# seryrzu/centroFlye

Measured on AMD Instinct MI355X. Metric: long-read bases/sec through rare-k-mer recruit+distance, higher is better.
Workload: dtype u8 bases -> u64 k-mers / u32 indices (integer only)

## Files before the change

### centroflye_amd/csrc/hip/cf_api.hip

```cpp
#include "cf_common.h"

#include <atomic>
#include <cstdlib>
#include <mutex>
#include <thread>

#ifndef CF_COPY_MODE_DEFAULT
#define CF_COPY_MODE_DEFAULT 1
#endif
struct alignas(16) cf_u32x4_api { uint32_t x, y, z, w; };

int cf_fail(cf_ctx* ctx, int code, const std::string& msg) {
    if (ctx) ctx->err = msg;
    return code;
}


static std::mutex g_pool_lock;
static std::vector<cf_ctx*> g_contexts;

static void cf_pool_flush_locked(cf_ctx* ctx) {
    for (auto& kv : ctx->pool) { ctx->block_bytes.erase(kv.second); (void)hipFree(kv.second); }
    ctx->pool.clear();
    ctx->pooled = 0;
// ... 457 lines not shown
        ctx->dist_hot_entries = (int)value;
    } else if (n == "lut_shift") {
        if (value < -1 || value > 3) return cf_fail(ctx, -22, "lut_shift out of range (-1 = by the set's size, 0 .. 3)");
        ctx->lut_shift = (int)value;
    } else if (n == "dist_regions") {
        if (value != 0 && value != 1 && value != 2 && value != 4 && value != 8) return cf_fail(ctx, -22, "dist_regions must be 0 (auto), 1, 2, 4 or 8");
        ctx->dist_regions = (int)value;
    } else if (n == "dist_dbits") {
        if (value != 0 && (value < 5 || value > 8)) return cf_fail(ctx, -22, "dist_dbits must be 0 (auto) or 5 .. 8");
        ctx->dist_dbits = (int)value;
    } else if (n == "dist_fill_pct") {
        if (value < 10 || value > 90) return cf_fail(ctx, -22, "dist_fill_pct out of range (10 .. 90)");
        ctx->dist_fill_pct = (int)value;
    } else if (n == "dist_edge_chunk") {
        if (value < 0 || value > (1 << 20)) return cf_fail(ctx, -22, "dist_edge_chunk out of range (0 = default, 1 .. 2^20)");
        ctx->dist_edge_chunk = (int)value;
    } else if (n == "dist_int_thr") {
        ctx->dist_int_thr = value != 0;
    } else if (n == "dist_sketch_bits") {
        if (value != 0 && value != 4 && value != 8) return cf_fail(ctx, -22, "dist_sketch_bits must be 0 (by min_cov), 4 or 8");
        ctx->dist_sketch_bits = (int)value;
    } else if (n == "dist_sketch_tail") {
        ctx->dist_sketch_tail = value != 0;
    } else if (n == "dist_classes") {
        ctx->dist_classes = value != 0;
    } else if (n == "dist_class_bits") {
        if (value < 1 || value > 16) return cf_fail(ctx, -22, "dist_class_bits out of range (1 .. 16)");
        ctx->dist_class_bits = (int)value;
    } else if (n == "dist_groups") {
        ctx->dist_groups = value != 0;
    } else if (n == "dist_group_cap") {
        if (value < 1 || value > 32) return cf_fail(ctx, -22, "dist_group_cap out of range (1 .. 32)");
        ctx->dist_group_cap = (int)value;
    } else if (n == "dist_sketch") {
        ctx->dist_sketch = value != 0;
    } else if (n == "dist_est_pct") {
        if (value < 5 || value > 100) return cf_fail(ctx, -22, "dist_est_pct out of range (5 .. 100)");
        ctx->dist_est_pct = (int)value;
    } else if (n == "dist_stage") {
        if (value < 0 || value > 2048) return cf_fail(ctx, -22, "dist_stage out of range (0 .. 2048)");
        ctx->dist_stage = (int)value;
    } else if (n == "place_fused") {
        ctx->place_fused = value != 0;
    } else if (n == "dist_region_bytes") {
        ctx->dist_region_bytes = value != 0;
    } else if (n == "place_mode") {
        if (value < 1 || value > 3) return cf_fail(ctx, -22, "place_mode out of range (1 = hash map, 2 = per-read regions unless min_inters < 4, 3 = per-read regions always)");
        ctx->place_mode = (int)value;
    } else if (n == "place_block") {
        if (value != 0 && (value < 128 || value > 1024 || value % 128)) return cf_fail(ctx, -22, "place_block must be 0 or a multiple of 128 in 128 .. 1024");
        ctx->place_block = (int)value;
    } else if (n == "place_row_words") {
        if (value != 0 && value != 32 && value != 64) return cf_fail(ctx, -22, "place_row_words must be 0 (auto), 32 or 64");
        ctx->place_row_words = (int)value;
    } else if (n == "place_l3") {
        if (value < 0 || value > 2) return cf_fail(ctx, -22, "place_l3 must be 0 (auto), 1 (always) or 2 (never)");
        ctx->place_l3 = (int)value;
    } else if (n == "place_l3_shift") {
        if (value < 0 || value > 6) return cf_fail(ctx, -22, "place_l3_shift must be 0 (= 6) .. 6");
        ctx->place_l3_shift = (int)value;
    } else if (n == "place_long_rescans") {
        if (value < -1 || value > 1000000) return cf_fail(ctx, -22, "place_long_rescans out of range (-1, 0 .. 1000000)");
        ctx->place_long_rescans = (int)value;
    } else if (n == "place_cmap_bits") {
        if (value < 0 || value > 30) return cf_fail(ctx, -22, "place_cmap_bits out of range (0 = default, 1 .. 30)");
        ctx->place_cmap_bits = (int)value;
// ... 85 lines not shown
```

### centroflye_amd/csrc/hip/cf_common.h

```cpp
#pragma once
#include <hip/hip_runtime.h>

#include <algorithm>
#include <cstdint>
#include <cstdio>
#include <cstring>
#include <map>
#include <string>
#include <unordered_map>
#include <vector>

#include "cfhip.h"

extern __shared__ __attribute__((aligned(16))) unsigned char cf_lds[];

#define CF_WAVE 64

#ifndef cf_lds_at
typedef __attribute__((address_space(3))) unsigned char cf_lds_u8;
__device__ __forceinline__ unsigned char* cf_lds_at(uint32_t off) { return (unsigned char*)((cf_lds_u8*)(uintptr_t)(off + 16u) - 16); }
__device__ __forceinline__ bool cf_lds_base_ok() { return (uint32_t)(uintptr_t)(cf_lds_u8*)cf_lds == 0u; }
#endif

__device__ __forceinline__ uint64_t cf_mix64(uint64_t x) {
// ... 114 lines not shown
    std::vector<cf_monodec_read> monodec_reads;
    std::vector<int64_t> monodec_ptr;
    std::vector<cf_monodec_inst> monodec_inst;
    cf_monodec_shape monodec_last{};

    static constexpr int kCopyThreads = 16;
    void* pin_slot[kCopyThreads] = {nullptr};
    hipStream_t pin_stream[kCopyThreads] = {nullptr};
    size_t pin_bytes = 0;
    int copy_threads = 16;

    cf_stats stats{};
    cf_times times{};

    int dist_block = 0;
    int dist_wgs = 0;
    int dist_slots = 0;
    int dist_wide = 0;
    int dist_post_atomics = 0;
    int dist_hot_cap = 0;
    int lut_shift = -1;
    int dist_hot_entries = 32768;
    int dist_regions = 0;
    int dist_region_bytes = 0;
    int dist_dbits = 0;
    int dist_fill_pct = 70;
    int dist_edge_chunk = 0;
    int dist_int_thr = 1;
    int dist_sketch = 1;
    bool dist_sketch_tail = true;
    int dist_class_bits = 16;
    bool dist_classes = true;
    bool dist_groups = true;
    int dist_group_cap = 32;
    int dist_sketch_bits = 0;
    int dist_est_pct = 80;
    int dist_stage = 2048;
    int place_chunk = 2, place_grid = 0;
    int place_fused = 1;
    int place_mode = 2;
    int place_block = 0;
    int place_row_words = 0;
    int place_long_rescans = 2;
    int place_cmap_bits = 0;
    int place_slots_per_unit = 0;
    int place_l3 = 0;
    int place_l3_shift = 0;
    int map_window = 0;
    int edit_lds_diags = 0;
    int tandem_key_mode = 0;
    int64_t tandem_batch_windows = 0;
    int64_t cons_batch_bytes = 0;
    int64_t ualign_batch_bytes = 0;
    int64_t monodec_batch_bytes = 0;
    int count_mode = 1;
    int count_bits = 0;
    int count_slots = 4096;
    int count_tile = 16;
    int count_skip_exotic = 0;
    int64_t comm_round_bytes = (int64_t)256 << 20;
    int comm_self_p2p = 0;
};

int cf_fail(cf_ctx* ctx, int code, const std::string& msg);
int cf_copy_h2d(cf_ctx* ctx, void* dev, const void* host, size_t bytes);
int cf_copy_d2h(cf_ctx* ctx, void* host, const void* dev, size_t bytes);
// ... 84 lines not shown
```

### centroflye_amd/csrc/hip/cf_dist.hip

```cpp
#include "cf_common.h"

#include <cstdlib>

void cf_free_edges(cf_ctx* c);
int cf_refresh_unique_count(cf_ctx* ctx);

#define DIST_STAGE_CAP 1024
#define DIST_STACK 112
#define DIST_UNROLL 4
#define DIST_ITEM (64u * DIST_UNROLL)
#define DIST_BM_BITS 65536u
#define DIST_HOT_CAP 2048u
#define DIST_EDGE_CHUNK 8192ull
#define DIST_OVQ 160u
#define DIST_LDS_HEAD (DIST_BM_BITS / 8 + 128)
#define DIST_CNT_MASK 0x7FFFFFu
#define DIST_SEL_BIT (1ull << 23)

#ifndef cf_ballot
__device__ __forceinline__ unsigned long long cf_ballot(bool p) { return __builtin_amdgcn_ballot_w64(p); }
#endif

struct alignas(16) cf_dist_rec { uint32_t e0; uint32_t len; uint32_t ig; uint32_t nu; };

__global__ void __launch_bounds__(256)
cf_post_hist_kernel(const int32_t* __restrict__ entries, int64_t e0, int64_t e1, uint32_t part, uint32_t n_parts, uint32_t* __restrict__ cnt) {
    const int64_t stride = (int64_t)gridDim.x * blockDim.x;
    for (int64_t i = e0 + (int64_t)blockIdx.x * blockDim.x + threadIdx.x; i < e1; i += stride) {
        const uint32_t x = (uint32_t)entries[i];
        if (n_parts == 1u || x % n_parts == part) atomicAdd(&cnt[x], 1u);
    }
}

__global__ void __launch_bounds__(256)
cf_post_fill_kernel(const int64_t* __restrict__ cloud_ptr, const int32_t* __restrict__ entries, int64_t u0, int64_t u1, uint32_t part, uint32_t n_parts,
                    const int64_t* __restrict__ post_ptr, uint32_t* __restrict__ cursor, int32_t* __restrict__ post,
                    uint32_t* __restrict__ first_unit) {
    const int lane = threadIdx.x & 63;
    const int64_t wave = ((int64_t)blockIdx.x * blockDim.x + threadIdx.x) >> 6;
    const int64_t n_waves = ((int64_t)gridDim.x * blockDim.x) >> 6;
    for (int64_t u = u0 + wave; u < u1; u += n_waves) {
        const int64_t a = cloud_ptr[u], b = cloud_ptr[u + 1];
        for (int64_t e = a + lane; e < b; e += 64) {
            const int32_t x = entries[e];
            if (n_parts != 1u && (uint32_t)x % n_parts != part) continue;
// ... 336 lines not shown
struct alignas(8) cf_dist_item { uint32_t e, m; };
#ifndef CF_DIST_ITEMS_BLOCKED
#define CF_DIST_ITEMS_BLOCKED 0
#endif
struct alignas(16) cf_dist_head { uint32_t a, n_items; unsigned long long ibase; uint32_t n_entries, n_useful, n_members, first_member; };

struct cf_dist_args {
    const int64_t* post_ptr;
    const int32_t* post;
    const int64_t* cloud_ptr;
    const int32_t* entries;
    const int32_t* unit_rend;
    const int32_t* unit_rbeg;
    const cf_dist_rec* urange;
    const uint16_t* entry_i;
    const uint8_t* entry_i8;
    uint32_t reg_shift;
    const uint32_t* packed;
    int64_t n_kmers;
    int32_t part, n_parts;
    int32_t min_d, max_d;
    uint32_t min_cov;
    double thr;
    uint32_t thr_num, thr_den;
    int32_t slots;
    uint32_t fill_limit;
    uint32_t est_limit;
    int32_t sketch;
    uint32_t sk_counters, sk_shift, sk_mask;
    uint32_t sk_fbits, sk_fsh, sk_wshift, sk_fmask, sk_guard, sk_bytes;
    const cf_dist_head* heads;
    const cf_dist_item* items;
    uint32_t stage_cap;
    uint32_t hot_cap;
    uint32_t hot_entries;
    uint32_t* edges;
    unsigned long long edge_cap;
    const uint32_t* member_mask;
    const int32_t* order;
    int64_t n_order;
    unsigned long long edge_chunk;
    unsigned long long* holes;
    unsigned long long* counters;
    uint32_t* unique_bits;
};

typedef uint32_t cf_raw4 __attribute__((ext_vector_type(4)));
struct __attribute__((packed, aligned(4))) cf_run4 { uint32_t x, y, z, w; };
__device__ __forceinline__ void cf_load_packed4(const cf_dist_args& A, uint32_t s_e, uint32_t l4, uint32_t& x, uint32_t& y, uint32_t& z, uint32_t& w) {
#if !defined(CF_NO_BUFFER_LOAD)
    const __amdgpu_buffer_rsrc_t rs = __builtin_amdgcn_make_buffer_rsrc((void*)A.packed, 0, (int)0xFFFFFFFFu, 0x00020000);
    const cf_raw4 v = __builtin_amdgcn_raw_buffer_load_b128(rs, (int)(l4 * 4u), (int)(s_e << 2), 0);
    x = v.x; y = v.y; z = v.z; w = v.w;
#else
    const uint32_t* p = A.packed + s_e;
    const cf_run4 r = *(const cf_run4*)(p + l4);
    x = r.x; y = r.y; z = r.z; w = r.w;
#endif
}

struct alignas(16) cf_u64x2 { unsigned long long x, y; };
struct alignas(16) cf_u32x4 { uint32_t x, y, z, w; };

template <int DB>
struct cf_tab_wide_t {
    static constexpr uint32_t kCntBits = 31 - DB, kCntMask = (1u << kCntBits) - 1u, kDMask = (1u << DB) - 1u, kDShift = 32 - DB;
// ... 451 lines not shown
        if (!(m.w[0] | m.w[1] | m.w[2] | m.w[3])) return;
        const bucket k = this->read(bk);
#pragma unroll
        for (int i = 0; i < 4; ++i) {
            const uint32_t cnt = cnt_of(m.w[i]);
            if (cnt >= min_cov && k.k[i] != kEmpty) {
                const uint32_t b = k.k[i] & kBMask;
                const unsigned long long total = (k.k[3] == kEmpty && N::home(N::hash(b), n_buckets) == bk) ? (unsigned long long)sum_of(k, m, b) : total_of(b, n_buckets);
                f(4u * bk + (uint32_t)i, b, k.k[i] >> kBBits, cnt, total);
            }
        }
    }
    static constexpr uint32_t kScanGroup = 4;
    static __device__ __forceinline__ uint32_t slot_of_bit(uint32_t bit) { return bit; }
    __device__ __forceinline__ uint32_t hot_mask(uint32_t g, uint32_t min_cov) const {
        const masks m = read_masks(g);
        const uint32_t need = max(min_cov, 1u);
        return (uint32_t)(all_of(m.w[0]) >= need) | ((uint32_t)(all_of(m.w[1]) >= need) << 1) | ((uint32_t)(all_of(m.w[2]) >= need) << 2) | ((uint32_t)(all_of(m.w[3]) >= need) << 3);
    }
    template <class F>
    __device__ __forceinline__ void eval_slot(uint32_t s, uint32_t n_buckets, uint32_t min_cov, F&& f) const {
        const uint32_t bk = s >> 2, i = s & 3u;
        const bucket k = this->read(bk);
        const masks m = read_masks(bk);
        uint32_t mine = k.k[0], mine_m = m.w[0];
#pragma unroll
        for (int j = 1; j < 4; ++j) { if (i == (uint32_t)j) { mine = k.k[j]; mine_m = m.w[j]; } }
        const uint32_t cnt = cnt_of(mine_m);
        if (mine == kEmpty || cnt < min_cov) return;
        const uint32_t b = mine & kBMask;
        const unsigned long long total = (k.k[3] == kEmpty && N::home(N::hash(b), n_buckets) == bk) ? (unsigned long long)sum_of(k, m, b) : total_of(b, n_buckets);
        f(s, b, mine >> kBBits, cnt, total);
    }
    template <class F>
    __device__ __forceinline__ void for_marked(uint32_t bk, F&& f) const {
        const uint32_t w = (mk[bk >> 3] >> ((bk & 7u) * 4u)) & 15u;
        if (!w) return;
        const bucket k = this->read(bk);
        const masks m = read_masks(bk);
#pragma unroll
        for (int i = 0; i < 4; ++i)
            if ((w >> i) & 1u) f(4u * bk + (uint32_t)i, k.k[i] & kBMask, k.k[i] >> kBBits, cnt_of(m.w[i]));
    }
    __device__ __forceinline__ void mark(uint32_t s) const { atomicOr(&mk[s >> 5], 1u << (s & 31u)); }
    __device__ __forceinline__ void unmark(uint32_t s) const { atomicAnd(&mk[s >> 5], ~(1u << (s & 31u))); }
};

struct cf_tab_region {
    static constexpr int PB = 4;
    static constexpr uint32_t kBBits = 24, kBMask = (1u << kBBits) - 1u;
    static constexpr uint32_t kSlotBytes = 6, kPerBucket = PB, kAll = (1u << PB) - 1u;
    static constexpr bool kMaskTab = false;
    static constexpr uint32_t kEmpty = 0xFFFFFFFFu;
    struct bucket { uint32_t k[PB]; };
    struct counts { uint32_t w[PB / 2]; };
    struct raw { uint32_t b, i; };
    typedef unsigned long long qitem;
    uint32_t* keys;
    uint32_t* cnt32;
    uint32_t S, nb_r;
    __device__ __forceinline__ void init(unsigned char* lds, uint32_t slots) { keys = (uint32_t*)lds; cnt32 = keys + slots; S = 0; nb_r = slots / PB; }
    __device__ __forceinline__ void configure(const cf_dist_args& A, uint32_t n_buckets) { S = A.reg_shift; nb_r = n_buckets >> A.reg_shift; }
    __device__ __forceinline__ void clear(uint32_t slots, uint32_t t, uint32_t nt) const {
        const cf_u32x4 e{kEmpty, kEmpty, kEmpty, kEmpty}, z{0u, 0u, 0u, 0u};
        for (uint32_t s = t; s < (slots >> 2); s += nt) ((cf_u32x4*)keys)[s] = e;
        for (uint32_t s = t; s < (slots >> 3); s += nt) ((cf_u32x4*)cnt32)[s] = z;
// ... 504 lines not shown
#ifndef CF_DIST_PF_B
#define CF_DIST_PF_B 1
#endif

#ifndef CF_DIST_LB_THREADS
#define CF_DIST_LB_THREADS 1024
#define CF_DIST_LB_BLOCKS 1
#endif
template <class Tab, bool CLS>
__global__ void __launch_bounds__(CF_DIST_LB_THREADS, CF_DIST_LB_BLOCKS) cf_dist_kernel(cf_dist_args A) {
    const int t = threadIdx.x, lane = t & 63, nt = blockDim.x;
    uint32_t* bm = (uint32_t*)cf_lds_at(0u);
    uint32_t* sh = bm + DIST_BM_BITS / 32;
    unsigned char* lds_tab = cf_lds_at(DIST_LDS_HEAD);
    Tab T;
    T.init(lds_tab, (uint32_t)A.slots);
    T.configure(A, (uint32_t)A.slots / Tab::kPerBucket);
    uint32_t* sk = (uint32_t*)lds_tab;
    size_t tab_bytes = (size_t)A.slots * Tab::kSlotBytes;
    if constexpr (Tab::kMaskTab) tab_bytes += Tab::extra_bytes((uint32_t)A.slots);
    uint16_t* stage = (uint16_t*)(lds_tab + tab_bytes);
    uint32_t* stack = (uint32_t*)(stage + DIST_STAGE_CAP + 8);
    typename Tab::qitem* wq0 = (typename Tab::qitem*)(stack + 2 * DIST_STACK);
    const uint32_t wv = (uint32_t)__builtin_amdgcn_readfirstlane((int)(t >> 6)), nw = (uint32_t)nt >> 6;
    typename Tab::qitem* wq = wq0 + (size_t)wv * DIST_QSTRIDE;
    typename Tab::qitem* ovq = wq0 + (size_t)(nt >> 6) * DIST_QSTRIDE + (size_t)wv * DIST_OVQ;
    uint16_t* hotl = (uint16_t*)(wq0 + (size_t)(nt >> 6) * (DIST_QSTRIDE + DIST_OVQ));
    uint8_t* wqb = (uint8_t*)(hotl + DIST_HOT_CAP) + (size_t)wv * (DIST_QSTRIDE + DIST_OVQ);
    uint8_t* ovqb = wqb + DIST_QSTRIDE;
    const uint32_t slots = (uint32_t)A.slots, n_buckets = slots / Tab::kPerBucket;
    unsigned long long acc_E = 0, acc_spill = 0, acc_pass = 0, acc_edges = 0;
#if defined(CF_DIST_DIAG_COUNT)
    unsigned long long dg_swept = 0;
    unsigned long long dg[8] = {0, 0, 0, 0, 0, 0, 0, 0};
#define CF_DG(X) X
#define CF_DG_PTR (&dg[0])
#else
#define CF_DG(X)
#define CF_DG_PTR nullptr
#endif
#if defined(CF_DIST_STAMPS)
    unsigned long long stamp_acc[8] = {0, 0, 0, 0, 0, 0, 0, 0}, stamp_t = __builtin_amdgcn_s_memtime();
#endif

    const int64_t q_per = (A.n_order + 7) / 8;
    auto pop_issue = [&]() -> unsigned long long { return atomicAdd(&A.counters[16 + 16 * (blockIdx.x & 7)], 1ull); };
    auto pop_finish = [&](unsigned long long q) -> long long {
        const int x0 = (int)(blockIdx.x & 7);
        const int64_t lo0 = x0 * q_per, hi0 = min((int64_t)(x0 + 1) * q_per, A.n_order);
        if (lo0 + (int64_t)q < hi0) return lo0 + (int64_t)q;
        for (int s8 = 1; s8 < 8; ++s8) {
            const int x = (int)((blockIdx.x + s8) & 7);
            const int64_t lo = x * q_per, hi = min((int64_t)(x + 1) * q_per, A.n_order);
            if (lo >= hi) continue;
            const unsigned long long q2 = atomicAdd(&A.counters[16 + 16 * x], 1ull);
            if (lo + (int64_t)q2 < hi) return lo + (int64_t)q2;
        }
        return -1;
    };
    long long nx_idx = -1;
    cf_dist_head nx_head{0u, 0u, 0ull, 0u, 0u, 1u, 0u};
    unsigned long long nx_q = 0;
    if (!cf_lds_base_ok()) { if (t == 0) atomicOr(&A.counters[4], 2ull); return; }
    auto publish_next = [&]() {
        sh[16] = (uint32_t)(unsigned long long)nx_idx; sh[17] = (uint32_t)((unsigned long long)nx_idx >> 32);
        sh[18] = nx_head.a; sh[19] = nx_head.n_items; sh[20] = (uint32_t)nx_head.ibase; sh[21] = (uint32_t)(nx_head.ibase >> 32);
// ... 90 lines not shown
                            for (int u = 0; u < DIST_UNROLL; ++u)
                                if (seen_[u] >= m_guard && ((ok >> u) & 1u)) atomicSub(&sk[sft_[u] >> 5], 1u << (sft_[u] & 31u));
                        }
                        if (seen_max == m_fmask) sh[m_flag] = 1u;
                    }
                    return false;
                });
                CF_STAMP(6);
            }
            __syncthreads();
            CF_STAMP(7);
            if (!sh[m_flag]) break;
            if (m_fbits == 8u) { mark_all = true; break; }
            m_fbits = 8u; m_fsh = 3u; m_wshift = 2u; m_fmask = 255u; m_guard = 0x7FFFFFFFu; m_shift = A.sk_shift + 1u; m_flag = 31u;
            }
        }
        if (t == 0) { nx_idx = pop_finish(nx_q); if (nx_idx >= 0) nx_head = A.heads[nx_idx]; }
        if (mark_all) {
            const cf_u32x4 ones{0xFFFFFFFFu, 0xFFFFFFFFu, 0xFFFFFFFFu, 0xFFFFFFFFu};
            for (uint32_t s = (uint32_t)t; s < DIST_BM_BITS / 128; s += (uint32_t)nt) ((cf_u32x4*)bm)[s] = ones;
            if (t == 0) {
                uint32_t P0 = 1;
                while (P0 < 64u && (unsigned long long)n_ent_a > (unsigned long long)A.est_limit * P0) P0 <<= 1;
                for (uint32_t i = 0; i < P0; ++i) { stack[2 * i] = P0; stack[2 * i + 1] = i; }
                sh[2] = P0;
                pop_pass();
            }
        }
        bool spilled = false;
        if (CF_DIST_ABL < 7) T.clear(slots, (uint32_t)t, (uint32_t)nt);
        __syncthreads();
        while (true) {
            const uint32_t P = sh[3], pidx = sh[4], pmask = P - 1u;
            uint32_t my_e = 0, s_e = 0;
            CF_STAMP(2);
            {
                uint32_t qtail = 0, otail = 0;
                bool too_full = sh[0] > A.fill_limit;
#if CF_DIST_HOTBLK
                uint32_t hcur = 0, hend = 0;
#define CF_DIST_HOT(SLOT) {                                                                                   \
                    const unsigned long long hm_ = cf_ballot((SLOT) != 0xFFFFFFFFu);                           \
                    if (hm_ && use_hot) {       \
                        const uint32_t hn_ = (uint32_t)__popcll(hm_), room_ = hend - hcur;                    \
                        uint32_t hp_ = hcur + cf_rank_in(hm_);                                                \
                        if (hn_ > room_) {       \
                            uint32_t nb_ = 0;                                                                 \
                            if (lane == 0) nb_ = atomicAdd(&sh[11], 64u);                                     \
                            nb_ = (uint32_t)__builtin_amdgcn_readfirstlane((int)nb_);                         \
                            if (nb_ + (uint32_t)lane < DIST_HOT_CAP) hotl[nb_ + (uint32_t)lane] = (uint16_t)0xFFFFu; \
                            hp_ = hp_ < hend ? hp_ : nb_ + (hp_ - hend);                                      \
                            hcur = nb_ + (hn_ - room_); hend = nb_ + 64u;                                     \
                        } else hcur += hn_;                                                                   \
                        if ((SLOT) != 0xFFFFFFFFu && hp_ < DIST_HOT_CAP) hotl[hp_] = (uint16_t)(SLOT);        \
                    }                                                                                         \
                }
#elif defined(CF_DIST_DIAG_NOHOT)
#define CF_DIST_HOT(SLOT) { if ((SLOT) == 0xFFFFFFF0u) sh[11] = 1u; }
#else
#define CF_DIST_HOT(SLOT) {                                                                                   \
                    const unsigned long long hm_ = cf_ballot((SLOT) != 0xFFFFFFFFu);                           \
                    if (hm_ && use_hot) {                                                                     \
                        uint32_t hb_ = 0;                                                                     \
                        if (lane == 0) hb_ = atomicAdd(&sh[11], (uint32_t)__popcll(hm_));                     \
                        hb_ = (uint32_t)__builtin_amdgcn_readfirstlane((int)hb_) + cf_rank_in(hm_);          \
                        if ((SLOT) != 0xFFFFFFFFu && hb_ < DIST_HOT_CAP) hotl[hb_] = (uint16_t)(SLOT);        \
// ... 201 lines not shown
            const uint32_t n_groups = slots / Tab::kScanGroup;
            for (uint32_t g0 = 0; g0 < n_groups; g0 += (uint32_t)nt) {
                const uint32_t bk = g0 + (uint32_t)t;
                const uint32_t m = bk < n_groups ? T.hot_mask(bk, A.min_cov) : 0u;
                const uint32_t cnt = (uint32_t)__popc(m);
                if (cf_ballot(cnt != 0u)) {
                    uint32_t total = 0;
                    for (uint32_t k = 0; k < Tab::kScanGroup; ++k) { const unsigned long long bk_ = cf_ballot(cnt > k); if (!bk_) break; total += (uint32_t)__popcll(bk_); }
                    uint32_t base = 0;
                    if (lane == 0) base = atomicAdd(&sh[11], total);
                    base = (uint32_t)__builtin_amdgcn_readfirstlane((int)base);
                    uint32_t mm = m;
                    for (uint32_t k = 0; k < Tab::kScanGroup; ++k) {
                        const unsigned long long bk_ = cf_ballot(cnt > k);
                        if (!bk_) break;
                        if (cnt > k) {
                            const uint32_t bit = (uint32_t)__ffs((int)mm) - 1u;
                            mm &= mm - 1u;
                            const uint32_t pos = base + cf_rank_in(bk_);
                            if (pos < hot_cap) hot[pos] = (uint16_t)(Tab::kScanGroup * bk + Tab::slot_of_bit(bit));
                        }
                        base += (uint32_t)__popcll(bk_);
                    }
                }
            }
            __syncthreads();
            }
            const uint32_t n_hot = sh[11];
            auto dominant = [&](uint32_t cnt, unsigned long long total) -> bool {
                if (A.thr_den) return (unsigned long long)A.thr_den * cnt >= (unsigned long long)A.thr_num * total;
                return ((double)cnt / (double)total) >= A.thr;
            };
            uint32_t sel_prev = 0, sp_left = 0;
            for (uint32_t mj = 0; mj < n_mem; ++mj) {
                const uint32_t am = mj ? (uint32_t)A.order[(size_t)m_first + mj] : a;
                if constexpr (Tab::kMaskTab) T.set_member(A.member_mask[(size_t)m_first + mj], T.counting);
                const unsigned long long ch_base = ((unsigned long long)sh[29] << 32) | sh[28];
                const uint32_t ch_rows = sh[27];
                auto put_row = [&](unsigned long long o, uint32_t b, uint32_t dd, uint32_t cnt) {
                    if (o < A.edge_cap) *(cf_u32x4*)(A.edges + 4 * o) = cf_u32x4{dd, am, b, cnt};
                    const uint32_t bit = 1u << (b & 31);
                    if (!(A.unique_bits[b >> 5] & bit)) atomicOr(&A.unique_bits[b >> 5], bit);
                };
                auto set_unique = [&](uint32_t w, uint32_t b) { const uint32_t bit = 1u << (b & 31); if (!(w & bit)) atomicOr(&A.unique_bits[b >> 5], bit); };
                auto keep = [&](bool sel, uint32_t s, uint32_t b, uint32_t dd, uint32_t cnt) -> bool {
                    const unsigned long long m = cf_ballot(sel);
                    if (!m) return false;
                    uint32_t row0 = 0;
                    if (lane == 0) { const uint32_t n = (uint32_t)__popcll(m); atomicAdd(&sh[8], n); row0 = atomicAdd(&sh[26], n); }
                    const uint32_t row = (uint32_t)__builtin_amdgcn_readfirstlane((int)row0) + (uint32_t)__popcll(m & lt);
                    const bool late = sel && row >= ch_rows;
                    const unsigned long long o = ch_base + row;
                    if (sel && !late && o < A.edge_cap) *(cf_u32x4*)(A.edges + 4 * o) = cf_u32x4{dd, am, b, cnt};
                    const unsigned long long ml = cf_ballot(late);
                    if (ml) {
                        uint32_t p0 = 0;
                        if (lane == 0) p0 = atomicAdd(&sh[30], (uint32_t)__popcll(ml));
                        const uint32_t pos = (uint32_t)__builtin_amdgcn_readfirstlane((int)p0) + (uint32_t)__popcll(ml & lt);
                        if (late) { T.mark(s); if (pos < A.stage_cap) stage[pos] = (uint16_t)s; }
                    }
                    return sel && !late;
                };
                if (CF_DIST_ABL >= 1) { }
                else if (n_hot <= hot_cap) {
                    bool p_on = false;
                    uint32_t p_w = 0, p_b = 0;
                    for (uint32_t i0 = 0; i0 < n_hot; i0 += (uint32_t)nt) {
                        const uint32_t i = i0 + (uint32_t)t;
                        bool sel = false;
                        uint32_t s = 0, eb = 0, ed = 0, ec = 0;
                        if (i < n_hot && (s = hot[i]) != 0xFFFFu) {
                            T.eval_slot(s, n_buckets, A.min_cov, [&](uint32_t, uint32_t b, uint32_t dd, uint32_t cnt, unsigned long long total) { sel = b != am && dominant(cnt, total); eb = b; ed = dd; ec = cnt; });
                        }
                        const bool wrote = keep(sel, s, eb, ed, ec);
                        uint32_t w_new = 0;
                        if (wrote) w_new = A.unique_bits[eb >> 5];
                        if (p_on) set_unique(p_w, p_b);
                        p_on = wrote; p_w = w_new; p_b = eb;
                    }
                    if (p_on) set_unique(p_w, p_b);
                } else {
                    for (uint32_t bk = (uint32_t)t; bk < n_buckets; bk += (uint32_t)nt)
                        T.for_counts_at_least(bk, n_buckets, A.min_cov, [&](uint32_t s, uint32_t b, uint32_t dd, uint32_t cnt, unsigned long long total) {
                            if (b != am && dominant(cnt, total)) {
                                atomicAdd(&sh[8], 1u);
                                const uint32_t row = atomicAdd(&sh[26], 1u);
                                if (row < ch_rows) put_row(ch_base + row, b, dd, cnt);
                                else {
                                    T.mark(s);
                                    const uint32_t pos = atomicAdd(&sh[30], 1u);
                                    if (pos < A.stage_cap) stage[pos] = (uint16_t)s;
                                }
                            }
                        });
                }
                __syncthreads();
                CF_STAMP(4);
                const uint32_t n_sel = sh[8] - sel_prev, n_late = sh[30];
                sel_prev += n_sel;
                sp_left = sh[2];
                if (t == 0) {
                    acc_E += sh[7];
                    if (mj == 0u) { ++acc_pass; CF_DG(dg_swept += sh[7];) }
                    if (n_sel) { acc_edges += n_sel; atomicOr(&A.unique_bits[am >> 5], 1u << (am & 31)); }
// ... 21 lines not shown
                if (mj + 1u < n_mem) {
                    __syncthreads();
                    if (n_late) {
                        for (uint32_t bk = (uint32_t)t; bk < n_buckets; bk += (uint32_t)nt) T.for_marked(bk, [&](uint32_t s, uint32_t, uint32_t, uint32_t) { T.unmark(s); });
                        __syncthreads();
                    }
                }
            }
            CF_STAMP(5);
            if (sp_left == 0u) break;
            __syncthreads();
            if (t == 0) pop_pass();
            T.clear(slots, (uint32_t)t, (uint32_t)nt);
            __syncthreads();
        }
        if (spilled && t == 0) ++acc_spill;
    }
    if (t == 0) {
        if (acc_E && !Tab::kMaskTab) atomicAdd(&A.counters[1], acc_E);
        if (acc_spill) atomicAdd(&A.counters[2], acc_spill);
        if (acc_pass) atomicAdd(&A.counters[5], acc_pass);
        if (acc_edges) atomicAdd(&A.counters[6], acc_edges);
        if (sh[27] > sh[26]) {
            const unsigned long long h = atomicAdd(&A.counters[7], 1ull), cb = ((unsigned long long)sh[29] << 32) | sh[28];
            A.holes[2 * h] = cb + sh[26]; A.holes[2 * h + 1] = (unsigned long long)(sh[27] - sh[26]);
        }
#if defined(CF_DIST_STAMPS)
        for (int i = 0; i < 8; ++i) atomicAdd(&A.counters[8 + i], stamp_acc[i]);
#endif
    }
#if defined(CF_DIST_DIAG_COUNT)
    for (int i = 0; i < 8; ++i) if (dg[i]) atomicAdd(&A.counters[8 + i], dg[i]);
    if (t == 0 && dg_swept) atomicAdd(&A.counters[147], dg_swept);
#endif
}

__global__ void __launch_bounds__(256)
cf_max_u32_kernel(const uint32_t* __restrict__ v, int64_t n, uint32_t* __restrict__ out) {
    uint32_t m = 0;
    const int64_t stride = (int64_t)gridDim.x * blockDim.x;
    for (int64_t i = (int64_t)blockIdx.x * blockDim.x + threadIdx.x; i < n; i += stride) m = max(m, v[i]);
    for (int d = 32; d >= 1; d >>= 1) m = max(m, __shfl_down(m, (unsigned)d));
    if ((threadIdx.x & 63) == 0 && m) atomicMax(out, m);
}

__global__ void __launch_bounds__(256)
cf_edge_compact_kernel(uint32_t* __restrict__ edges, const unsigned long long* __restrict__ src_start, const unsigned long long* __restrict__ src_pre, int n_src,
                       const unsigned long long* __restrict__ dst_start, const unsigned long long* __restrict__ dst_pre, int n_dst, unsigned long long n_move) {
    const unsigned long long stride = (unsigned long long)gridDim.x * blockDim.x;
    for (unsigned long long k = (unsigned long long)blockIdx.x * blockDim.x + threadIdx.x; k < n_move; k += stride) {
        int lo = 0, hi = n_src - 1;
        while (lo < hi) { const int mid = (lo + hi) >> 1; if (src_pre[mid] > k) hi = mid; else lo = mid + 1; }
        const unsigned long long from = src_start[lo] + (k - (lo ? src_pre[lo - 1] : 0ull));
        lo = 0; hi = n_dst - 1;
        while (lo < hi) { const int mid = (lo + hi) >> 1; if (dst_pre[mid] > k) hi = mid; else lo = mid + 1; }
        const unsigned long long to = dst_start[lo] + (k - (lo ? dst_pre[lo - 1] : 0ull));
        *(cf_u32x4*)(edges + 4 * to) = *(const cf_u32x4*)(edges + 4 * from);
    }
}

__global__ void __launch_bounds__(256)
cf_edge_checksum_kernel(const uint32_t* __restrict__ edges, int64_t n, unsigned long long* __restrict__ out) {
    unsigned long long s = 0;
    const int64_t stride = (int64_t)gridDim.x * blockDim.x;
    for (int64_t i = (int64_t)blockIdx.x * blockDim.x + threadIdx.x; i < n; i += stride) {
        const cf_u32x4 e = *(const cf_u32x4*)(edges + 4 * i);
// ... 40 lines not shown
    if (v_n_entries >= ((int64_t)1 << 32) - 8 * (int64_t)DIST_ITEM) return cf_fail(ctx, -34, "cf_dist_edges: more than 2^32 cloud entries (the sweeps address them with 32-bit indices)");
    if (edge_cap < 0) edge_cap = 0;
    const int64_t R = gv ? ctx->g_reads : ctx->n_reads, U = gv ? ctx->g_units : ctx->n_units, K = ctx->n_kmers;
    CF_HIP(hipSetDevice(ctx->device));
    CF_HIP(hipEventRecord(ctx->ev0, ctx->stream));
    if (min_n < 0) min_n = 0;
    if (max_n > R) max_n = R;
    if (max_n < min_n) max_n = min_n;
    if (min_n > R) min_n = R;
    const int64_t u0 = v_h_unit_ptr[(size_t)min_n], u1 = v_h_unit_ptr[(size_t)max_n];
    const int32_t min_d_eff = min_d < 1 ? 1 : min_d;

    uint32_t *d_pcnt = nullptr, *d_cursor = nullptr, *d_first = nullptr;
    unsigned long long *d_okeys = nullptr, *d_otmp = nullptr;
    int32_t* d_order = nullptr;
    int64_t n_order = 0, n_item_slots = 0;
    uint32_t *d_icnt = nullptr, *d_ialloc = nullptr;
    int64_t* d_ibase = nullptr;
    cf_dist_head* d_heads = nullptr;
    cf_dist_item* d_items = nullptr;
    unsigned long long* d_holes = nullptr;
    int64_t n_stored = 0;
    int64_t* d_post_ptr = nullptr;
    int32_t *d_post = nullptr, *d_rend = nullptr, *d_rbeg = nullptr;
    uint16_t* d_entry_i = nullptr;
    uint32_t* d_packed = nullptr;
    cf_dist_rec* d_urange = nullptr;
    bool narrow = false, wide16 = false, region = false, region26 = false;
    int narrow_db = 8, reg_shift = 0;
    uint8_t* d_entry_i8 = nullptr;
    unsigned long long* d_cnt = nullptr;
    int64_t n_post = 0;
    unsigned long long h_cnt[8] = {0};
    const size_t n_cnt = 8 + 16 * 9;
    const int max_blocks = std::max(1, ctx->n_cu) * 8;
    cf_free_edges(ctx);
    cf_scratch tmp(ctx);
    CF_TRY(tmp.get(&d_pcnt, (size_t)K + 1, "posting counts"));
    CF_TRY(tmp.get(&d_cursor, (size_t)K + 1, "posting cursors"));
    CF_TRY(tmp.get(&d_post_ptr, (size_t)K + 1, "posting offsets"));
    CF_TRY(tmp.get(&d_rend, (size_t)U + 1, "unit read ends"));
    CF_TRY(tmp.get(&d_rbeg, (size_t)U + 1, "unit read begins"));
    CF_TRY(tmp.get(&d_urange, (size_t)U + 1, "unit partner ranges"));
    CF_TRY(tmp.get(&d_cnt, n_cnt, "dist counters"));
    CF_TRY(tmp.get(&d_first, (size_t)K + 1, "first posting units"));
    CF_HIP(hipMemsetAsync(d_pcnt, 0, (size_t)(K + 1) * 4, ctx->stream));
    CF_HIP(hipMemsetAsync(d_cursor, 0, (size_t)(K + 1) * 4, ctx->stream));
    CF_HIP(hipMemsetAsync(d_cnt, 0, n_cnt * 8, ctx->stream));
    CF_HIP(hipMemsetAsync(d_first, 0xFF, (size_t)(K + 1) * 4, ctx->stream));
    int64_t e0 = 0, e1 = 0;
    CF_HIP(hipMemcpy(&e0, v_cloud_ptr + u0, 8, hipMemcpyDeviceToHost));
    CF_HIP(hipMemcpy(&e1, v_cloud_ptr + u1, 8, hipMemcpyDeviceToHost));
    const bool by_sort = !ctx->dist_post_atomics && e1 > e0 && (e1 - e0) < ((int64_t)1 << 32) && U < ((int64_t)1 << 31);
    if (by_sort) {
        int64_t n = e1 - e0;
        const int64_t K_part = (K + n_parts - 1) / n_parts;
        int kb = 1; while (kb < 32 && ((int64_t)1 << kb) < std::max<int64_t>(K_part, 2)) ++kb;
        kb = (kb + 7) & ~7;
        const unsigned g_units = (unsigned)cf_grid_for((u1 - u0) * 64, 256, max_blocks);
        {
            cf_scratch recs(ctx);
            unsigned long long *d_recs = nullptr, *d_rtmp = nullptr, *d_sorted = nullptr;
            uint32_t* d_ucnt = nullptr; int64_t* d_uoff = nullptr;
            if (n_parts > 1) {
                CF_TRY(recs.get(&d_ucnt, (size_t)(u1 - u0) + 1, "kept entries per unit"));
                CF_TRY(recs.get(&d_uoff, (size_t)(u1 - u0) + 1, "record offsets per unit"));
                CF_HIP(hipMemsetAsync(d_ucnt + (u1 - u0), 0, 4, ctx->stream));
// ... 44 lines not shown
    int need_bits = 1; while (((int64_t)1 << need_bits) <= d_need) ++need_bits;
    wide16 = d_need > 255;
    int kb = 24; while (kb < 32 && K >= ((int64_t)1 << kb) - 1) ++kb;
    narrow_db = 32 - kb;
    if (ctx->dist_dbits) narrow_db = std::min(narrow_db, ctx->dist_dbits);
    const bool stream4_ok = v_n_entries + (int64_t)DIST_ITEM < ((int64_t)1 << 30);
    narrow = !wide16 && !ctx->dist_wide && narrow_db >= 5 && narrow_db >= need_bits && max_post <= 32767u && stream4_ok;
    if (ctx->dist_dbits && !narrow) return cf_fail(ctx, -22, "cf_dist_edges: dist_dbits does not fit this input (distances or k-mer ranks need more bits)");
    if (!narrow || ctx->dist_regions) {
        reg_shift = 0;
        while (reg_shift < 3 && ((K - 1) >> reg_shift) > ((int64_t)1 << 24) - 2) ++reg_shift;
        if (ctx->dist_regions) { int want = 0; while ((1 << want) < ctx->dist_regions) ++want; reg_shift = std::max(reg_shift, want); }
        region = !wide16 && !ctx->dist_wide && !ctx->dist_dbits && reg_shift <= 3 && ((K - 1) >> reg_shift) <= ((int64_t)1 << 24) - 2 && max_post <= 32767u && K < ((int64_t)1 << 31);
        if (ctx->dist_regions && !region) return cf_fail(ctx, -22, "cf_dist_edges: dist_regions does not fit this input");
        if (region) narrow = false;
        region26 = region && !ctx->dist_region_bytes && K <= ((int64_t)1 << 26) && d_need <= 127 && stream4_ok;
    }
    const bool groups_fit = CF_DIST_HAS_GROUPS && ctx->dist_groups && ctx->dist_classes && by_sort && narrow && ctx->dist_sketch && min_cov >= 2 && min_cov <= 200;
    if (max_post >= (1u << 23) || (wide16 && max_post > 32767u)) return cf_fail(ctx, -34, wide16 ? "cf_dist_edges: distances above 255 with a k-mer of more than 32767 postings" : "cf_dist_edges: a k-mer has more than 2^23 postings");
    if (narrow || region26) { CF_TRY(tmp.get(&d_packed, (size_t)v_n_entries + DIST_ITEM, "packed cloud entries")); }
    else if (region) { CF_TRY(tmp.get(&d_entry_i8, (size_t)v_n_entries + 4 * DIST_ITEM, "entry unit indices (bytes)")); }
    else CF_TRY(tmp.get(&d_entry_i, (size_t)v_n_entries + 1, "entry unit indices"));
    if (U && v_n_entries)
        hipLaunchKernelGGL(cf_entry_unit_kernel, dim3((unsigned)cf_grid_for(U * 64, 256, max_blocks)), dim3(256), 0, ctx->stream,
                           v_cloud_ptr, (const int32_t*)d_rbeg, v_entries, U, d_entry_i, d_packed, region26 ? 26 : 32 - narrow_db, d_entry_i8, d_cnt + 144);
    CF_KERNEL_CHECK("the postings kernels");
    CF_HIP(hipEventRecord(ctx->ev2, ctx->stream));

    cf_dist_args A;
    A.post_ptr = d_post_ptr; A.post = d_post; A.cloud_ptr = v_cloud_ptr; A.entries = v_entries; A.unit_rend = d_rend; A.unit_rbeg = d_rbeg; A.urange = d_urange; A.entry_i = d_entry_i; A.packed = d_packed; A.entry_i8 = d_entry_i8; A.reg_shift = (uint32_t)reg_shift;
    A.n_kmers = K; A.part = part; A.n_parts = n_parts; A.min_d = min_d_eff; A.max_d = max_d; A.min_cov = min_cov; A.thr = rel_threshold;
    A.thr_num = (rel_threshold == 0.8 && ctx->dist_int_thr) ? 4u : 0u; A.thr_den = A.thr_num ? 5u : 0u;
    A.stage_cap = (uint32_t)std::min(ctx->dist_stage, DIST_STAGE_CAP);
    A.hot_cap = ctx->dist_hot_cap > 0 ? (uint32_t)ctx->dist_hot_cap : 0xFFFFFFFFu;
    A.hot_entries = ctx->dist_hot_entries >= 0 ? (uint32_t)ctx->dist_hot_entries : 0xFFFFFFFFu;
    double per_first = 0.0;
    if (n_post && u1 > u0) {
        unsigned long long partner_units = 0;
        for (int64_t r = min_n; r < max_n; ++r) {
            const int64_t nu = v_h_unit_ptr[(size_t)r + 1] - v_h_unit_ptr[(size_t)r];
            const int64_t span = (int64_t)max_d - min_d_eff + 1;
            if (nu <= min_d_eff || span <= 0) continue;
            const int64_t full = std::max<int64_t>(0, nu - max_d);
            const int64_t tail = nu - min_d_eff - full;
            partner_units += (unsigned long long)(full * span) + (unsigned long long)(tail > 0 ? tail * (tail + 1) / 2 : 0);
        }
        const double cloud = (double)(e1 - e0) / (double)(u1 - u0), post_per_unit = (double)n_post / (double)(u1 - u0);
        per_first = (double)partner_units * cloud * post_per_unit / (double)std::max<int64_t>(1, (K - part + n_parts - 1) / n_parts);
    }
    const bool groups = groups_fit && per_first <= 32768.0;
    const uint32_t slot_bytes = groups ? cf_tab_mask<8>::kSlotBytes : (narrow || region) ? cf_tab_narrow::kSlotBytes : cf_tab_wide::kSlotBytes;
    int wgs = ctx->dist_wgs, block = ctx->dist_block;
    if (wgs == 0) wgs = (block > 512 || per_first > 32768.0) ? 1 : 2;
    if (block == 0) block = wgs == 1 ? 1024 : 512;
    const size_t qitem_bytes = narrow ? sizeof(cf_tab_narrow::qitem) : sizeof(cf_tab_wide::qitem);
    const size_t lds_fixed = DIST_LDS_HEAD + (size_t)(2 * DIST_STACK) * 4 + DIST_STAGE_CAP * 2 + 16 + (size_t)(block / 64) * (DIST_QSTRIDE + DIST_OVQ) * qitem_bytes + DIST_HOT_CAP * 2
                             + (groups ? (((size_t)(block / 64) * (DIST_QSTRIDE + DIST_OVQ) + 15) & ~(size_t)15) : 0);
    const int64_t budget8 = ((int64_t)160 * 1024 / wgs - (int64_t)lds_fixed) / 8;
    if (budget8 < 256) return cf_fail(ctx, -22, "cf_dist_edges: dist_wgs leaves no LDS for the table");
    if (ctx->dist_slots > budget8) return cf_fail(ctx, -22, "cf_dist_edges: dist_slots does not fit the 160 KiB LDS next to the work lists");
    const int64_t slots8 = ctx->dist_slots ? ctx->dist_slots : budget8;
    A.slots = (int32_t)((slots8 * 8 / slot_bytes) & ~(region ? (int64_t)(32 << reg_shift) - 1 : 7ll));
    if (groups) {
        A.slots = (int32_t)((slots8 * 8 / cf_tab_mask<8>::kSlotBytes) & ~7ll);
        while (A.slots > 8 && (int64_t)A.slots * cf_tab_mask<8>::kSlotBytes + cf_tab_mask<8>::extra_bytes((uint32_t)A.slots) > slots8 * 8) A.slots -= 8;
    }
// ... 98 lines not shown
    void (*kern)(cf_dist_args) = classes ? CF_DIST_KERN(true) : CF_DIST_KERN(false);
#if CF_DIST_HAS_GROUPS
    if (groups) kern = narrow_db == 8 ? cf_dist_kernel<cf_tab_mask<8>, true> : narrow_db == 7 ? cf_dist_kernel<cf_tab_mask<7>, true> : narrow_db == 6 ? cf_dist_kernel<cf_tab_mask<6>, true> : cf_dist_kernel<cf_tab_mask<5>, true>;
#endif
#undef CF_DIST_KERN
    CF_HIP(hipFuncSetAttribute((const void*)kern, hipFuncAttributeMaxDynamicSharedMemorySize, (int)lds));
    {
        A.edge_chunk = ctx->dist_edge_chunk > 0 ? (unsigned long long)ctx->dist_edge_chunk : DIST_EDGE_CHUNK;
        const int64_t rows = edge_cap > 0 ? edge_cap + (int64_t)grid * (int64_t)A.edge_chunk : 0;
        CF_TRY(cf_alloc_t(ctx, &ctx->d_edges, (size_t)rows * 4, "edges"));
        ctx->edge_cap = rows;
        A.edges = ctx->d_edges; A.edge_cap = (unsigned long long)rows;
    }
    CF_TRY(tmp.get(&d_holes, 2 * ((size_t)grid + 1), "edge holes"));
    A.holes = d_holes;
    CF_HIP(hipMemsetAsync(d_cnt + 6, 0, 16, ctx->stream));
    if (n_a > 0 && max_d >= min_d_eff && n_post > 0) {
        hipLaunchKernelGGL(kern, dim3((unsigned)grid), dim3((unsigned)block), lds, ctx->stream, A);
        CF_KERNEL_CHECK("cf_dist_kernel");
    }
    CF_HIP(hipEventRecord(ctx->ev3, ctx->stream));
    CF_HIP(hipMemcpyAsync(h_cnt, d_cnt, 64, hipMemcpyDeviceToHost, ctx->stream));
    CF_HIP(hipEventRecord(ctx->ev1, ctx->stream));
    CF_HIP(hipEventSynchronize(ctx->ev1));
#if defined(CF_DIST_DIAG_COUNT)
    {
        unsigned long long st[8];
        if (hipMemcpy(st, d_cnt + 8, 64, hipMemcpyDeviceToHost) == hipSuccess)
            std::fprintf(stderr, "[cf_dist diag] parked-insert loop trips=%llu overflow calls=%llu parked inserts run=%llu drains=%llu inserts drained=%llu cycles(sum over waves): parked runs=%llu drains=%llu table sweeps=%llu; waves=%d passes=%llu\n", st[0], st[1], st[2], st[3], st[4], st[5], st[6], st[7], grid * (block / 64), h_cnt[5]);
        unsigned long long su[4], up[2] = {0, 0};
        const bool have_up = groups && hipMemcpy(up, d_cnt + 148, 16, hipMemcpyDeviceToHost) == hipSuccess;
        if (hipMemcpy(su, d_cnt + 144, 32, hipMemcpyDeviceToHost) == hipSuccess)
            std::fprintf(stderr, "[cf_dist diag] sketch items=%llu of items=%llu (rows are sets=%d) classes=%lld members=%lld entries swept=%llu of %llu per member\n", su[1], su[2], su[0] ? 0 : 1, have_up ? (long long)up[1] : (long long)n_heads, (long long)n_order, su[3], h_cnt[1]);
        if (have_up)
            std::fprintf(stderr, "[cf_dist diag] groups=%lld members=%lld union postings=%llu slots=%d split groups=%llu\n", (long long)n_heads, (long long)n_order, up[0], (int)A.slots, h_cnt[2]);
    }
#endif
#if defined(CF_DIST_STAMPS)
    {
        unsigned long long st[8];
        if (hipMemcpy(st, d_cnt + 8, 64, hipMemcpyDeviceToHost) == hipSuccess)
            std::fprintf(stderr, "[cf_dist stamps] pop=%llu prologue=%llu sketch=%llu clear=%llu stream=%llu filter=%llu write=%llu sweep_end_wait=%llu (shader cycles summed over %d workgroups; passes=%llu)\n",
                         st[0], st[1], st[6], st[2], st[3], st[4], st[5], st[7], grid, h_cnt[5]);
    }
#endif
    if (h_cnt[4] & 4ull) return cf_fail(ctx, -5, "cf_dist_edges: internal error, a group's union has more postings than its mask has bits");
    if (h_cnt[4] & 2ull) return cf_fail(ctx, -5, "cf_dist_edges: the kernel's dynamic LDS does not begin at address 0");
    if (h_cnt[4]) return cf_fail(ctx, -34, "cf_dist_edges: (b,d) table could not be partitioned far enough");
    {
        const unsigned long long a_cap = std::min<unsigned long long>(h_cnt[0], A.edge_cap);
        std::vector<unsigned long long> hh(2 * (size_t)h_cnt[7]);
        if (!hh.empty()) {
            CF_HIP(hipMemcpyAsync(hh.data(), d_holes, hh.size() * 8, hipMemcpyDeviceToHost, ctx->stream));
            CF_HIP(hipStreamSynchronize(ctx->stream));
        }
        std::vector<std::pair<unsigned long long, unsigned long long>> holes;
        for (size_t i = 0; i + 1 < hh.size(); i += 2) {
            const unsigned long long s0 = std::min(hh[i], a_cap), s1 = std::min(hh[i] + hh[i + 1], a_cap);
            if (s1 > s0) holes.emplace_back(s0, s1);
        }
        std::sort(holes.begin(), holes.end());
        unsigned long long hole_rows = 0;
        for (auto& h : holes) hole_rows += h.second - h.first;
        const unsigned long long n_valid = a_cap - hole_rows;
        n_stored = (int64_t)std::min<unsigned long long>(n_valid, (unsigned long long)edge_cap);
        std::vector<unsigned long long> dst_start, dst_pre, src_start, src_pre;
// ... 44 lines not shown
```

Measured before the change: 4.295 billion.

## Filter hot slots against all group members in one pass with register-cached keys

Adds a default-on path for mask-table groups. Each hot slot's bucket keys and the masks of its probe chain are read once into registers (up to 8 keys). All group members are then evaluated against them in batches of 32 via readlane, with edges written through LDS-coordinated chunk allocation. Before, the code looped over members, set the member mask, and re-walked each slot's probe chain to compute totals. The new path adds extra barriers per member batch, holds more registers per lane, and falls back to total_of for slots that overflow the register capacity.

```diff
diff --git a/centroflye_amd/csrc/hip/cf_api.hip b/centroflye_amd/csrc/hip/cf_api.hip
--- a/centroflye_amd/csrc/hip/cf_api.hip
+++ b/centroflye_amd/csrc/hip/cf_api.hip
@@ -513,6 +513,8 @@
     } else if (n == "dist_group_cap") {
         if (value < 1 || value > 32) return cf_fail(ctx, -22, "dist_group_cap out of range (1 .. 32)");
         ctx->dist_group_cap = (int)value;
+    } else if (n == "dist_filter_once") {
+        ctx->dist_filter_once = value != 0;
     } else if (n == "dist_sketch") {
         ctx->dist_sketch = value != 0;
     } else if (n == "dist_est_pct") {
diff --git a/centroflye_amd/csrc/hip/cf_common.h b/centroflye_amd/csrc/hip/cf_common.h
--- a/centroflye_amd/csrc/hip/cf_common.h
+++ b/centroflye_amd/csrc/hip/cf_common.h
@@ -170,6 +170,7 @@
     int dist_class_bits = 16;
     bool dist_classes = true;
     bool dist_groups = true;
+    bool dist_filter_once = true;
     int dist_group_cap = 32;
     int dist_sketch_bits = 0;
     int dist_est_pct = 80;
diff --git a/centroflye_amd/csrc/hip/cf_dist.hip b/centroflye_amd/csrc/hip/cf_dist.hip
--- a/centroflye_amd/csrc/hip/cf_dist.hip
+++ b/centroflye_amd/csrc/hip/cf_dist.hip
@@ -11,6 +11,7 @@
 #define DIST_ITEM (64u * DIST_UNROLL)
 #define DIST_BM_BITS 65536u
 #define DIST_HOT_CAP 2048u
+#define DIST_MEMBER_KEYS 8
 #define DIST_EDGE_CHUNK 8192ull
 #define DIST_OVQ 160u
 #define DIST_LDS_HEAD (DIST_BM_BITS / 8 + 128)
@@ -413,6 +414,7 @@
     const cf_dist_head* heads;
     const cf_dist_item* items;
     uint32_t stage_cap;
+    uint32_t filter_once;
     uint32_t hot_cap;
     uint32_t hot_entries;
     uint32_t* edges;
@@ -930,6 +932,23 @@
         const unsigned long long total = (k.k[3] == kEmpty && N::home(N::hash(b), n_buckets) == bk) ? (unsigned long long)sum_of(k, m, b) : total_of(b, n_buckets);
         f(s, b, mine >> kBBits, cnt, total);
     }
+#if defined(CF_DIST_DIAG_COUNT)
+    __device__ __forceinline__ uint32_t diag_walk(uint32_t s, uint32_t n_buckets, uint32_t min_cov) const {
+        const uint32_t bk0 = s >> 2, i = s & 3u;
+        const bucket k0 = this->read(bk0);
+        const uint32_t mine = k0.k[i];
+        if (mine == kEmpty || cnt_of(msk[s]) < min_cov) return 0u;
+        const uint32_t b = mine & kBMask;
+        if (k0.k[3] == kEmpty && N::home(N::hash(b), n_buckets) == bk0) return 0u;
+        uint32_t bk = N::home(N::hash(b), n_buckets), n = 0;
+        for (uint32_t probe = 0; probe < n_buckets; ++probe) {
+            ++n;
+            if (this->read(bk).k[3] == kEmpty) break;
+            bk = bk + 1 == n_buckets ? 0u : bk + 1;
+        }
+        return n;
+    }
+#endif
     template <class F>
     __device__ __forceinline__ void for_marked(uint32_t bk, F&& f) const {
         const uint32_t w = (mk[bk >> 3] >> ((bk & 7u) * 4u)) & 15u;
@@ -1500,6 +1519,7 @@
     unsigned long long acc_E = 0, acc_spill = 0, acc_pass = 0, acc_edges = 0;
 #if defined(CF_DIST_DIAG_COUNT)
     unsigned long long dg_swept = 0;
+    unsigned long long dg_hot = 0, dg_hot_mem = 0, dg_walks = 0, dg_walk_bk = 0, dg_ovf = 0;
     unsigned long long dg[8] = {0, 0, 0, 0, 0, 0, 0, 0};
 #define CF_DG(X) X
 #define CF_DG_PTR (&dg[0])
@@ -1656,6 +1676,7 @@
         __syncthreads();
         while (true) {
             const uint32_t P = sh[3], pidx = sh[4], pmask = P - 1u;
+            if constexpr (Tab::kMaskTab) { if (t == 0) { ((uint32_t*)stage)[0] = 0u; ((uint32_t*)stage)[3] = 0u; } }
             uint32_t my_e = 0, s_e = 0;
             CF_STAMP(2);
             {
@@ -1923,6 +1944,132 @@
                 return ((double)cnt / (double)total) >= A.thr;
             };
             uint32_t sel_prev = 0, sp_left = 0;
+            CF_DG(if (t == 0) { dg_hot += n_hot; dg_hot_mem += (unsigned long long)n_hot * n_mem; })
+            bool once = false;
+            if constexpr (Tab::kMaskTab) once = A.filter_once != 0u && n_hot <= hot_cap && CF_DIST_ABL < 1;
+            if constexpr (Tab::kMaskTab) if (once) {
+                uint32_t* cw = (uint32_t*)stage;
+                unsigned long long ch_base = ((unsigned long long)sh[29] << 32) | sh[28];
+                uint32_t ch_rows = sh[27], cur = sh[26], batch = 0;
+                const bool counting = T.counting;
+                auto cntf = [&](uint32_t w, uint32_t M) -> uint32_t { return counting ? w : (uint32_t)__popc(w & M); };
+                bool p_on = false;
+                uint32_t p_w = 0, p_b = 0;
+                auto set_unique = [&](uint32_t w, uint32_t b) { const uint32_t bit = 1u << (b & 31); if (!(w & bit)) atomicOr(&A.unique_bits[b >> 5], bit); };
+                for (uint32_t i0 = 0; i0 < n_hot; i0 += (uint32_t)nt) {
+                    const uint32_t i = i0 + (uint32_t)t;
+                    bool act = false, ovf = false;
+                    uint32_t b = 0, dd = 0, mine_m = 0, s = 0xFFFFu;
+                    uint32_t w[DIST_MEMBER_KEYS];
+#pragma unroll
+                    for (int q = 0; q < DIST_MEMBER_KEYS; ++q) w[q] = 0u;
+                    if (i < n_hot) s = hot[i];
+                    if (s != 0xFFFFu) {
+                        const uint32_t bk = s >> 2, si = s & 3u;
+                        const typename Tab::bucket k = T.read(bk);
+                        const typename Tab::masks m = T.read_masks(bk);
+                        uint32_t mine = k.k[0];
+                        mine_m = m.w[0];
+#pragma unroll
+                        for (int j = 1; j < 4; ++j) { if (si == (uint32_t)j) { mine = k.k[j]; mine_m = m.w[j]; } }
+                        if (mine != Tab::kEmpty && T.all_of(mine_m) >= A.min_cov) {
+                            act = true; b = mine & Tab::kBMask; dd = mine >> Tab::kBBits;
+                            if (k.k[3] == Tab::kEmpty && Tab::N::home(Tab::N::hash(b), n_buckets) == bk) {
+#pragma unroll
+                                for (int j = 0; j < 4; ++j) w[j] = ((k.k[j] & Tab::kBMask) == b && k.k[j] != Tab::kEmpty) ? m.w[j] : 0u;
+                            } else {
+                                uint32_t n_w = 0, cb = Tab::N::home(Tab::N::hash(b), n_buckets);
+                                for (uint32_t probe = 0; probe < n_buckets; ++probe) {
+                                    const typename Tab::bucket k2 = T.read(cb);
+                                    CF_DG(++dg_walk_bk;)
+                                    const typename Tab::masks m2 = T.read_masks(cb);
+#pragma unroll
+                                    for (int j = 0; j < 4; ++j)
+                                        if ((k2.k[j] & Tab::kBMask) == b && k2.k[j] != Tab::kEmpty) {
+#pragma unroll
+                                            for (int q = 0; q < DIST_MEMBER_KEYS; ++q) w[q] = n_w == (uint32_t)q ? m2.w[j] : w[q];
+                                            ++n_w;
+                                        }
+                                    if (k2.k[3] == Tab::kEmpty) break;
+                                    cb = cb + 1 == n_buckets ? 0u : cb + 1;
+                                }
+                                ovf = n_w > (uint32_t)DIST_MEMBER_KEYS;
+                                CF_DG(++dg_walks; dg_ovf += (unsigned long long)ovf;)
+                            }
+                        }
+                    }
+                    for (uint32_t j0 = 0; j0 < n_mem; j0 += 32u, ++batch) {
+                        const uint32_t nbm = min(32u, n_mem - j0), c = batch % 3u, cn = (batch + 1u) % 3u;
+                        uint32_t Mv = 0, Av = 0;
+                        if ((uint32_t)lane < nbm) { Mv = A.member_mask[(size_t)m_first + j0 + (uint32_t)lane]; Av = (j0 + (uint32_t)lane) ? (uint32_t)A.order[(size_t)m_first + j0 + (uint32_t)lane] : a; }
+                        uint32_t selbits = 0, wave_n = 0, wave_mem = 0;
+                        for (uint32_t jj = 0; jj < nbm; ++jj) {
+                            const uint32_t M = (uint32_t)__builtin_amdgcn_readlane((int)Mv, (int)jj), aj = (uint32_t)__builtin_amdgcn_readlane((int)Av, (int)jj);
+                            const uint32_t cnt = cntf(mine_m, M);
+                            bool sel = false;
+                            if (act && cnt >= A.min_cov && b != aj) {
+                                unsigned long long total = 0;
+                                if (ovf) { T.set_member(M, counting); total = T.total_of(b, n_buckets); }
+                                else {
+#pragma unroll
+                                    for (int q = 0; q < DIST_MEMBER_KEYS; ++q) total += cntf(w[q], M);
+                                }
+                                sel = dominant(cnt, total);
+                            }
+                            const unsigned long long bal = cf_ballot(sel);
+                            selbits |= (uint32_t)sel << jj;
+                            wave_n += (uint32_t)__popcll(bal);
+                            wave_mem |= (uint32_t)(bal != 0ull) << jj;
+                        }
+                        uint32_t rel0 = 0;
+                        if (lane == 0 && wave_n) { rel0 = atomicAdd(&cw[c], wave_n); atomicOr(&cw[3u + c], wave_mem); }
+                        if (t == 0) { cw[cn] = 0u; cw[3u + cn] = 0u; }
+                        __syncthreads();
+                        rel0 = (uint32_t)__builtin_amdgcn_readfirstlane((int)rel0);
+                        const uint32_t tot = cw[c], end = cur + tot;
+                        unsigned long long nbase = 0;
+                        if (end > ch_rows) {
+                            if (t == 0) {
+                                const unsigned long long take = ((unsigned long long)(end - ch_rows) + A.edge_chunk - 1ull) / A.edge_chunk * A.edge_chunk;
+                                const unsigned long long nb = atomicAdd(&A.counters[0], take);
+                                sh[28] = (uint32_t)nb; sh[29] = (uint32_t)(nb >> 32); sh[27] = (uint32_t)take;
+                            }
+                            __syncthreads();
+                            nbase = ((unsigned long long)sh[29] << 32) | sh[28];
+                        }
+                        if ((uint32_t)t < nbm && ((cw[3u + c] >> t) & 1u)) atomicOr(&A.unique_bits[Av >> 5], 1u << (Av & 31u));
+                        if (t == 0) acc_edges += tot;
+                        if (wave_n) {
+                            uint32_t run = cur + rel0;
+                            for (uint32_t jj = 0; jj < nbm; ++jj) {
+                                const bool bit = ((selbits >> jj) & 1u) != 0u;
+                                const unsigned long long bal = cf_ballot(bit);
+                                if (!bal) continue;
+                                const uint32_t M = (uint32_t)__builtin_amdgcn_readlane((int)Mv, (int)jj), aj = (uint32_t)__builtin_amdgcn_readlane((int)Av, (int)jj);
+                                if (bit) {
+                                    const uint32_t r = run + (uint32_t)__popcll(bal & lt);
+                                    const unsigned long long o = r < ch_rows ? ch_base + r : nbase + (r - ch_rows);
+                                    if (o < A.edge_cap) *(cf_u32x4*)(A.edges + 4 * o) = cf_u32x4{dd, aj, b, cntf(mine_m, M)};
+                                }
+                                run += (uint32_t)__popcll(bal);
+                            }
+                        }
+                        if (p_on) set_unique(p_w, p_b);
+                        p_on = selbits != 0u;
+                        if (p_on) { p_w = A.unique_bits[b >> 5]; p_b = b; }
+                        if (end > ch_rows) { cur = end - ch_rows; ch_base = nbase; ch_rows = sh[27]; } else cur = end;
+                    }
+                }
+                if (p_on) set_unique(p_w, p_b);
+                if (n_hot == 0u) __syncthreads();
+                sp_left = sh[2];
+                if (t == 0) {
+                    sh[26] = cur; sh[27] = ch_rows;
+                    ++acc_pass; CF_DG(dg_swept += sh[7];)
+                }
+                CF_STAMP(4);
+            }
+            if (!once)
             for (uint32_t mj = 0; mj < n_mem; ++mj) {
                 const uint32_t am = mj ? (uint32_t)A.order[(size_t)m_first + mj] : a;
                 if constexpr (Tab::kMaskTab) T.set_member(A.member_mask[(size_t)m_first + mj], T.counting);
@@ -1961,6 +2108,7 @@
                         bool sel = false;
                         uint32_t s = 0, eb = 0, ed = 0, ec = 0;
                         if (i < n_hot && (s = hot[i]) != 0xFFFFu) {
+                            if constexpr (Tab::kMaskTab) { CF_DG(const uint32_t wb_ = T.diag_walk(s, n_buckets, A.min_cov); dg_walks += (unsigned long long)(wb_ != 0u); dg_walk_bk += wb_;) }
                             T.eval_slot(s, n_buckets, A.min_cov, [&](uint32_t, uint32_t b, uint32_t dd, uint32_t cnt, unsigned long long total) { sel = b != am && dominant(cnt, total); eb = b; ed = dd; ec = cnt; });
                         }
                         const bool wrote = keep(sel, s, eb, ed, ec);
@@ -2048,6 +2196,9 @@
 #if defined(CF_DIST_DIAG_COUNT)
     for (int i = 0; i < 8; ++i) if (dg[i]) atomicAdd(&A.counters[8 + i], dg[i]);
     if (t == 0 && dg_swept) atomicAdd(&A.counters[147], dg_swept);
+    for (int d = 32; d >= 1; d >>= 1) { dg_walks += __shfl_down(dg_walks, (unsigned)d); dg_walk_bk += __shfl_down(dg_walk_bk, (unsigned)d); dg_ovf += __shfl_down(dg_ovf, (unsigned)d); }
+    if (lane == 0 && dg_walks) { atomicAdd(&A.counters[154], dg_walks); atomicAdd(&A.counters[155], dg_walk_bk); if (dg_ovf) atomicAdd(&A.counters[156], dg_ovf); }
+    if (t == 0 && dg_hot) { atomicAdd(&A.counters[152], dg_hot); atomicAdd(&A.counters[153], dg_hot_mem); }
 #endif
 }
 
@@ -2154,7 +2305,7 @@
     unsigned long long* d_cnt = nullptr;
     int64_t n_post = 0;
     unsigned long long h_cnt[8] = {0};
-    const size_t n_cnt = 8 + 16 * 9;
+    const size_t n_cnt = 8 + 16 * 9 + 5;
     const int max_blocks = std::max(1, ctx->n_cu) * 8;
     cf_free_edges(ctx);
     cf_scratch tmp(ctx);
@@ -2265,6 +2416,7 @@
     A.n_kmers = K; A.part = part; A.n_parts = n_parts; A.min_d = min_d_eff; A.max_d = max_d; A.min_cov = min_cov; A.thr = rel_threshold;
     A.thr_num = (rel_threshold == 0.8 && ctx->dist_int_thr) ? 4u : 0u; A.thr_den = A.thr_num ? 5u : 0u;
     A.stage_cap = (uint32_t)std::min(ctx->dist_stage, DIST_STAGE_CAP);
+    A.filter_once = ctx->dist_filter_once ? 1u : 0u;
     A.hot_cap = ctx->dist_hot_cap > 0 ? (uint32_t)ctx->dist_hot_cap : 0xFFFFFFFFu;
     A.hot_entries = ctx->dist_hot_entries >= 0 ? (uint32_t)ctx->dist_hot_entries : 0xFFFFFFFFu;
     double per_first = 0.0;
@@ -2429,6 +2581,9 @@
         const bool have_up = groups && hipMemcpy(up, d_cnt + 148, 16, hipMemcpyDeviceToHost) == hipSuccess;
         if (hipMemcpy(su, d_cnt + 144, 32, hipMemcpyDeviceToHost) == hipSuccess)
             std::fprintf(stderr, "[cf_dist diag] sketch items=%llu of items=%llu (rows are sets=%d) classes=%lld members=%lld entries swept=%llu of %llu per member\n", su[1], su[2], su[0] ? 0 : 1, have_up ? (long long)up[1] : (long long)n_heads, (long long)n_order, su[3], h_cnt[1]);
+        unsigned long long mf[5];
+        if (hipMemcpy(mf, d_cnt + 152, 40, hipMemcpyDeviceToHost) == hipSuccess)
+            std::fprintf(stderr, "[cf_dist diag] member filter: n_hot=%llu n_hot x members=%llu eval_slot calls with total_of=%llu buckets read in total_of=%llu slots with more keys than registers=%llu\n", mf[0], mf[1], mf[2], mf[3], mf[4]);
         if (have_up)
             std::fprintf(stderr, "[cf_dist diag] groups=%lld members=%lld union postings=%llu slots=%d split groups=%llu\n", (long long)n_heads, (long long)n_order, up[0], (int)A.slots, h_cnt[2]);
     }
```

New measurement: 4.864 billion, median of 6. +13.2%, better.
